# HasnainRaz/Fast-SRGAN

Hardware: AMD Instinct MI355X
Metric: SR train-step images/sec (96->384 4x, full GAN step: G+D+VGG perceptual loss) (higher is better)
Workload: dtype x3v; 1 GPU; BASELINE configs[2]: full GAN training step, 8 residual blocks / 64 filters, 96x96->384x384; per_gpu_batch=32, global_batch=32, parallelism=dp1, collectives=none, rccl_world_size=1, launch=hipGraph replay

## Files before the change

fast-srgan_amd/_lib.py:

```python
import ctypes
import os

_HERE = os.path.dirname(os.path.abspath(__file__))
LIB_PATH = os.environ.get("FSR_HIP_LIB") or os.path.join(_HERE, "libfsr_hip.so")

FSR_F32, FSR_BF16, FSR_F16, FSR_X3 = 0, 1, 2, 3
ACT_NONE, ACT_RELU, ACT_LEAKY, ACT_PRELU, ACT_TANH = 0, 1, 2, 3, 4
CONV_FWD, CONV_DGRAD = 0, 1
PACK_FWD, PACK_FWD_PS, PACK_DGRAD, PACK_DGRAD_PS = 0, 1, 2, 3
OUT_DTYPE, OUT_F32, OUT_U8, OUT_I420, OUT_NV12 = 0, 1, 2, 3, 4
YUV_BT601, YUV_BT709 = 0, 1
SITING_JPEG, SITING_MPEG2 = 0, 1
CHROMA_420, CHROMA_422, CHROMA_444 = 0, 1, 2
LAYOUT_PLANAR, LAYOUT_NV12 = 0, 1
BLUR_MAX_RADIUS, BLUR_TAPS = 9, 19
QUALITY_Y, QUALITY_RGB = 0, 1
OPT_BIAS, OPT_PRELU, OPT_OSCALE, OPT_MASK, OPT_PREACT, OPT_STATS = 1, 2, 4, 8, 16, 32
ABI_VERSION = 16

c_int, c_float, c_void_p, c_size_t, c_ll = ctypes.c_int, ctypes.c_float, ctypes.c_void_p, ctypes.c_size_t, ctypes.c_longlong


class ConvDesc(ctypes.Structure):
    _fields_ = [
# ... 44 lines not shown
    "fsr_i420_to_image_deep": (c_int, [P, P, c_int, c_int, c_int, c_int, c_int, c_int, c_int, P]),
    "fsr_image_to_i420": (c_int, [P, c_int, c_int, c_int, c_int, c_int, c_int, P, P]),
    "fsr_resample_image_i420_deep": (c_int, [P, c_int, c_int, c_int, c_int, c_int, P, P, P, c_int, P, P, P, c_int, c_int, c_int, c_int, P, P]),
    "fsr_yuv_to_image": (c_int, [P, P, c_int, c_int, c_int, c_int, c_int, c_int, c_int, c_int, P]),
    "fsr_image_to_yuv": (c_int, [P, c_int, c_int, c_int, c_int, c_int, c_int, c_int, P, P]),
    "fsr_resample_image_yuv": (c_int, [P, c_int, c_int, c_int, c_int, c_int, P, P, P, c_int, P, P, P, c_int, c_int, c_int, c_int, c_int, P, P]),
    "fsr_yuv_to_image_ex": (c_int, [P, P, c_int, c_int, c_int, c_int, c_int, c_int, c_int, c_int, c_int, P]),
    "fsr_image_to_yuv_ex": (c_int, [P, c_int, c_int, c_int, c_int, c_int, c_int, c_int, c_int, P, P]),
    "fsr_resample_image_yuv_ex": (c_int, [P, c_int, c_int, c_int, c_int, c_int, P, P, P, c_int, P, P, P, c_int, c_int, c_int, c_int, c_int, c_int,
                                          P, P]),
    "fsr_resample_image": (c_int, [P, c_int, c_int, c_int, c_int, c_int, P, P, P, c_int, P, P, P, c_int, c_int, c_int, c_int, P, P]),
    "fsr_pack_conv3x3_c3": (c_int, [c_int, P, c_int, P, c_int, P]),
    "fsr_tanh_bwd_image": (c_int, [P, c_ll, c_ll, c_ll, c_ll, P, c_int, c_int, c_int, P, P, P, P]),
    "fsr_conv3x3_c3_fwd": (c_int, [c_int, P, c_ll, c_ll, c_ll, c_ll, c_int, c_int, c_int, c_float, c_float, c_float, c_float,
                                   c_float, c_float, P, P, c_int, c_float, P, c_int, P, P, P, P]),
    "fsr_conv3x3_c3_wgrad_workspace": (ctypes.c_size_t, [c_int, c_int, c_int, c_int]),
    "fsr_conv3x3_c3_wgrad": (c_int, [c_int, P, c_ll, c_ll, c_ll, c_ll, c_int, c_int, c_int, c_float, c_float, c_float,
                                     c_float, c_float, c_float, P, c_int, P, P, P, c_int, P]),
    "fsr_tanh_bwd_scratch": (c_size_t, []),
    "fsr_tanh_bwd_to_nhwc": (c_int, [c_int, P, c_ll, c_ll, c_ll, c_ll, P, c_int, c_int, c_int, P, c_int, P, P, P]),
    "fsr_maxpool2_fwd": (c_int, [c_int, P, P, P, c_int, c_int, c_int, c_int, P]),
    "fsr_png_to_npy": (c_int, [P, P, c_int, c_int, P]),
    "fsr_png_decode_chw": (c_int, [ctypes.c_char_p, P, c_size_t, P, P]),
    "fsr_maxpool2_bwd_argmax": (c_int, [c_int, P, P, P, c_int, c_int, c_int, c_int, c_int, P]),
    "fsr_maxpool2_bwd": (c_int, [c_int, P, P, P, P, c_int, c_int, c_int, c_int, c_int, P]),
    "fsr_conv1x1_c1_fwd": (c_int, [c_int, P, P, P, P, c_int, c_int, P]),
    "fsr_conv1x1_c1_bwd_scratch": (c_size_t, [c_int]),
    "fsr_conv1x1_c1_bwd": (c_int, [c_int, P, P, P, P, P, P, P, c_int, c_int, P]),
    "fsr_loss_scratch": (c_size_t, []),
    "fsr_bce_logits_fwd": (c_int, [P, P, P, P, c_ll, P]),
# ... 66 lines not shown
```

fast-srgan_amd/csrc/conv_c3.hip:

```cpp
#include "fsr_common.h"
#include "fsr_host.h"

namespace {

struct C3Args {
  const float* img;
  long long sn, sc, sh, sw;
  int N, H, W;
  float scale[3], shift[3];
  const void* wpk;
  const float* bias;
  const float* prelu;
  int act;
  float slope;
  int cout;
  void* out;
  void* preact;
  unsigned char* signs;
  const void* dz;
  float* ws;
  int tiles_x, tiles_y, tiles_per_slab, ntiles;
};

constexpr int PW = 18;

__device__ __forceinline__ int patch_off(int k) {
  const int tap = k / 3, ci = k - tap * 3;
  return ((tap / 3) * PW + (tap % 3)) * 3 + ci;
}

template <typename T> __device__ __forceinline__ float round_T(float v);
template <> __device__ __forceinline__ float round_T<float>(float v) { return v; }
template <> __device__ __forceinline__ float round_T<bf16_t>(float v) { return bf2f(f2bf(v)); }
template <> __device__ __forceinline__ float round_T<f16_t>(float v) { return (float)(f16_t)v; }

#ifndef FSR_ABLC3
#define FSR_ABLC3 0
#endif
constexpr int C3_ABL = FSR_ABLC3;
#if FSR_ABLC3
#define C3_KEEP(v) asm volatile("" ::"v"(v))
#else
#define C3_KEEP(v) ((void)0)
#endif

template <int TH> struct PatchRegs {
  static constexpr int PN = (TH + 2) * PW * 3;
  static constexpr int PPT = (PN + 255) / 256;
  float v[PPT];
  unsigned okmask;
};
template <int TH>
__device__ __forceinline__ void patch_load(const C3Args& a, PatchRegs<TH>& r, int n, int y0, int x0, int tid) {
  const float* src = a.img + n * a.sn;
// ... 47 lines not shown
    const bool ok = i < PN && y >= 0 && y < a.H && x >= 0 && x < a.W;
    okmask |= (ok ? 1u : 0u) << j;
    if constexpr ((C3_ABL & 8) != 0) v[j] = (float)(i & 15);
    else v[j] = src[ok ? ci * a.sc + y * a.sh + x * a.sw : 0];
  }
#pragma unroll
  for (int j = 0; j < PPT; ++j) {
    const int i = tid + j * 256;
    const int ci = i % 3;
    const float sc = ci == 0 ? a.scale[0] : (ci == 1 ? a.scale[1] : a.scale[2]);
    const float sh = ci == 0 ? a.shift[0] : (ci == 1 ? a.shift[1] : a.shift[2]);
    if (i < PN) patch[i] = ((okmask >> j) & 1u) ? round_T<T>(v[j] * sc + sh) : 0.f;
  }
}

template <typename T, typename ST = T, int ROWS = 16>
__global__ __launch_bounds__(256) void conv_c3_fwd_kernel(const C3Args a) {
  constexpr int TH = ROWS, RPW = ROWS / 4;
  constexpr int PN = (TH + 2) * PW * 3, PPT = (PN + 255) / 256;
  constexpr bool STRIP = ROWS > 16;
  static_assert(ROWS == 16 || ROWS == 32 || ROWS == 64, "strip height");
  __shared__ float patch[PN];
  const int tid = threadIdx.x, lane = tid & 63, wave = __builtin_amdgcn_readfirstlane(tid >> 6);
  const int l15 = lane & 15, lg = lane >> 4;
  int bid = blockIdx.x;
  const int tx = bid % a.tiles_x;
  bid /= a.tiles_x;
  const int ty = bid % a.tiles_y;
  const int n = bid / a.tiles_y;
  const int nb = blockIdx.y;
  const int ntile = (a.cout - nb * 64 >= 64) ? 4 : (a.cout - nb * 64) / 16;
// ... 15 lines not shown
      if constexpr ((C3_ABL & 8) != 0) pv[j] = (float)(i & 15);
      else pv[j] = src[ok ? (unsigned)ci * usc + (unsigned)y * ush + (unsigned)x * usw : 0u];
    }
  }

  const T* wpk = (const T*)a.wpk;
  int koff[8];
  if constexpr (sizeof(T) == 2) {
#pragma unroll
    for (int e = 0; e < 8; ++e) koff[e] = (8 * lg + e < 27) ? patch_off(8 * lg + e) : -1;
  } else {
#pragma unroll
    for (int j = 0; j < 8; ++j) koff[j] = (lg + 4 * j < 27) ? patch_off(lg + 4 * j) : -1;
  }
  constexpr bool X3 = std::is_same<ST, x3_t>::value;
  const bool wide = (sizeof(T) == 2 || X3) && ntile == 4;
  s16x8 wf16[4];
  float wf32[4][8];
#pragma unroll
  for (int t = 0; t < 4; ++t) {
    if (t < ntile) {
      const int ch = wide ? (t >> 1) * 32 + (l15 >> 2) * 8 + (t & 1) * 4 + (l15 & 3) : t * 16 + l15;
      const T* row = wpk + (size_t)(nb * 64 + ch) * 32;
      if constexpr ((C3_ABL & 16) != 0) {
        if constexpr (sizeof(T) == 2) {
          wf16[t] = (s16x8){(short)lane, (short)t, 1, 2, 3, 4, 5, 6};
        } else {
#pragma unroll
          for (int j = 0; j < 8; ++j) wf32[t][j] = (float)(lane + j);
        }
      } else if constexpr (sizeof(T) == 2) {
        wf16[t] = *(const s16x8*)(row + 8 * lg);
      } else {
#pragma unroll
        for (int j = 0; j < 8; ++j) wf32[t][j] = row[lg + 4 * j];
      }
    }
  }
  float slope = (a.act == FSR_ACT_PRELU) ? a.prelu[0] : a.slope;
  if (a.act == FSR_ACT_NONE) slope = 1.f;
  if (a.act == FSR_ACT_RELU) slope = 0.f;
  f32x4 bv[4];
#pragma unroll
  for (int i = 0; i < 4; ++i) bv[i] = (f32x4){0.f, 0.f, 0.f, 0.f};
  auto load_bias = [&]() {
    if (a.bias) {
      if (wide) {
#pragma unroll
        for (int p = 0; p < 2; ++p) {
          bv[2 * p] = *(const f32x4*)(a.bias + nb * 64 + p * 32 + lg * 8);
          bv[2 * p + 1] = *(const f32x4*)(a.bias + nb * 64 + p * 32 + lg * 8 + 4);
        }
      } else {
#pragma unroll
        for (int t = 0; t < 4; ++t)
          if (t < ntile) bv[t] = *(const f32x4*)(a.bias + nb * 64 + t * 16 + lg * 4);
// ... 19 lines not shown
  if constexpr (!STRIP) load_bias();
#pragma unroll 1
  for (int m0 = 0; m0 < RPW; m0 += 4) {
    int mo = m0;
    if constexpr (STRIP) {
      FSR_TOUCH(mo);
      mo = __builtin_amdgcn_readfirstlane(mo);
    }
#pragma unroll
  for (int m = 0; m < 4; ++m) {
    const int r = wave * RPW + mo + m;
    const int gy = ty * TH + r;
    if constexpr (STRIP) {
      if (gy >= a.H) break;
    }
    const float* base = patch + (r * PW + l15) * 3;
    float xv[8];
#pragma unroll
    for (int e = 0; e < 8; ++e) xv[e] = koff[e] >= 0 ? base[koff[e]] : 0.f;
    s16x8 xf16;
    if constexpr (sizeof(T) == 2) {
      const unsigned p0 = pack2<T>(xv[0], xv[1]), p1 = pack2<T>(xv[2], xv[3]);
      const unsigned p2 = pack2<T>(xv[4], xv[5]), p3 = pack2<T>(xv[6], xv[7]);
      xf16 = __builtin_bit_cast(s16x8, (u32x4){p0, p1, p2, p3});
    }
    if constexpr (sizeof(T) == 2) {
      if (wide) {
        f32x4 acc[4];
#pragma unroll
        for (int t = 0; t < 4; ++t) {
// ... 3 lines not shown
        if (gx < a.W && gy < a.H) {
          const size_t off = (((size_t)n * a.H + gy) * a.W + gx) * a.cout + nb * 64 + lg * 8;
#pragma unroll
          for (int p = 0; p < 2; ++p) {
            f32x4 lo = acc[2 * p], hi = acc[2 * p + 1];
            lo += bv[2 * p];
            hi += bv[2 * p + 1];
            if (prep)
              fsr_st<4>((u32x4*)((T*)prep + off + p * 32), (u32x4)((u32x4){pack2<T>(lo[0], lo[1]), pack2<T>(lo[2], lo[3]),
                                                       pack2<T>(hi[0], hi[1]), pack2<T>(hi[2], hi[3])}));
#pragma unroll
            for (int q = 0; q < 4; ++q) {
              lo[q] = fmaxf(lo[q], 0.f) + slope * fminf(lo[q], 0.f);
              hi[q] = fmaxf(hi[q], 0.f) + slope * fminf(hi[q], 0.f);
            }
            const u32x4 pk = (u32x4){pack2<T>(lo[0], lo[1]), pack2<T>(lo[2], lo[3]), pack2<T>(hi[0], hi[1]), pack2<T>(hi[2], hi[3])};
            if constexpr ((C3_ABL & 1) != 0) C3_KEEP(pk);
            else fsr_st<4>((u32x4*)((T*)outp + off + p * 32), pk);
            if (a.signs) {
              unsigned b = 0u;
#pragma unroll
              for (int q = 0; q < 4; ++q) b |= ((int)(pk[q] << 16) > 0 ? 1u << (2 * q) : 0u) | ((int)(pk[q] & 0xffff0000u) > 0 ? 2u << (2 * q) : 0u);
              a.signs[(((size_t)n * a.H + gy) * a.W + gx) * (a.cout >> 3) + nb * 8 + p * 4 + lg] = (unsigned char)b;
            }
          }
        }
        continue;
      }
    }
    if constexpr (X3) {
      if (wide) {
// ... 4 lines not shown
#pragma unroll
          for (int j = 0; j < 8; ++j) {
            if constexpr ((C3_ABL & 2) != 0) acc[t][j & 3] += wf32[t][j] + xv[j];
            else acc[t] = mfma_f32_16x16x4(wf32[t][j], xv[j], acc[t]);
          }
        }
        if (gx < a.W && gy < a.H) {
          const size_t off = (((size_t)n * a.H + gy) * a.W + gx) * a.cout + nb * 64 + lg * 8;
#pragma unroll
          for (int p = 0; p < 2; ++p) {
            const f32x4 lo = acc[2 * p] + bv[2 * p], hi = acc[2 * p + 1] + bv[2 * p + 1];
            float v8[8] = {lo[0], lo[1], lo[2], lo[3], hi[0], hi[1], hi[2], hi[3]};
            if (prep) V16<x3_t, 4>::st((x3_t*)prep + off + p * 32, v8);
#pragma unroll
            for (int q = 0; q < 8; ++q) v8[q] = fmaxf(v8[q], 0.f) + slope * fminf(v8[q], 0.f);
            if constexpr ((C3_ABL & 1) != 0) {
#pragma unroll
              for (int q = 0; q < 8; ++q) C3_KEEP(v8[q]);
            } else {
              V16<x3_t, 4>::st((x3_t*)outp + off + p * 32, v8);
            }
            if (a.signs) {
              unsigned b = 0u;
#pragma unroll
              for (int q = 0; q < 4; ++q) {
                const unsigned hh = pack_bf16x2(v8[2 * q], v8[2 * q + 1]);
                b |= ((int)(hh << 16) > 0 ? 1u << (2 * q) : 0u) | ((int)(hh & 0xffff0000u) > 0 ? 2u << (2 * q) : 0u);
              }
              a.signs[(((size_t)n * a.H + gy) * a.W + gx) * (a.cout >> 3) + nb * 8 + p * 4 + lg] = (unsigned char)b;
            }
// ... 33 lines not shown
          if constexpr (sizeof(T) == 2) {
            u32x2 pk;
            pk.x = pack2<T>(acc[0], acc[1]);
            pk.y = pack2<T>(acc[2], acc[3]);
            fsr_st<4>((u32x2*)((T*)outp + off), (u32x2)(pk));
          } else if constexpr (std::is_same<ST, x3_t>::value) {
            x3_st4(outp + off, acc);
          } else {
            *(f32x4*)(outp + off) = acc;
          }
        }
      }
    });
  }
  }
}

template <typename T, typename ST = T>
__global__ __launch_bounds__(256) void conv_c3_wgrad_kernel(const C3Args a) {
  constexpr int TH = 8;
  constexpr bool F32 = sizeof(T) == 4;
  constexpr int PA = F32 ? 64 : 64 + 16;
  constexpr int PN = (TH + 2) * PW * 3;
  __shared__ float patch[PN];
  __shared__ __attribute__((aligned(16))) T dzt[TH * 16 * PA];
  const int tid = threadIdx.x, lane = tid & 63, wave = __builtin_amdgcn_readfirstlane(tid >> 6);
  const int l15 = lane & 15, lg = lane >> 4;
  const int slab = blockIdx.x, nb = blockIdx.y;
  const int cvalid = a.cout - nb * 64;
  const bool active = wave * 16 < cvalid;
  const ST* dzg = (const ST*)a.dz;
// ... 194 lines not shown
  }
  if (dtype != FSR_X3 || preact) return 16;
  const long long tiles_x = (w + 15) / 16;
  for (int rows = 64; rows > 16; rows >>= 1) {
    const long long strips = (h + rows - 1) / rows;
    if (tiles_x * strips * n >= C3_FWD_MIN_ROUNDS * C3_FWD_SLOTS && (strips * rows - h) * C3_FWD_MAX_PAD <= h) return rows;
  }
  return 16;
}

template <typename T, typename ST>
void c3_fwd_launch(int rows, dim3 grid, hipStream_t stream, const C3Args& a) {
  if (rows == 64) hipLaunchKernelGGL((conv_c3_fwd_kernel<T, ST, 64>), grid, dim3(256), 0, stream, a);
  else if (rows == 32) hipLaunchKernelGGL((conv_c3_fwd_kernel<T, ST, 32>), grid, dim3(256), 0, stream, a);
  else hipLaunchKernelGGL((conv_c3_fwd_kernel<T, ST, 16>), grid, dim3(256), 0, stream, a);
}

}

extern "C" int fsr_pack_conv3x3_c3(int dtype, const float* w_oihw, int cout, void* packed, int transposed, fsr_stream_t stream_) {
  if (!w_oihw || !packed || cout <= 0) return fsr_fail(-1, "fsr_pack_conv3x3_c3: bad argument");
  const int rows_pad = (cout + 15) / 16 * 16;
  const int blocks = (rows_pad * 32 + 255) / 256;
  if (dtype == FSR_BF16)
    hipLaunchKernelGGL(pack_c3_kernel<bf16_t>, dim3(blocks), dim3(256), 0, (hipStream_t)stream_, w_oihw, (bf16_t*)packed, cout, rows_pad, transposed);
  else if (dtype == FSR_F16)
    hipLaunchKernelGGL(pack_c3_kernel<f16_t>, dim3(blocks), dim3(256), 0, (hipStream_t)stream_, w_oihw, (f16_t*)packed, cout, rows_pad, transposed);
  else if (dtype == FSR_F32 || dtype == FSR_X3)
    hipLaunchKernelGGL(pack_c3_kernel<float>, dim3(blocks), dim3(256), 0, (hipStream_t)stream_, w_oihw, (float*)packed, cout, rows_pad, transposed);
  else
// ... 23 lines not shown
  a.signs = (unsigned char*)signs;
  const int rows = c3_fwd_rows(dtype, preact != nullptr, n, h, w, sc, sh, sw);
  a.tiles_x = (w + 15) / 16;
  a.tiles_y = (h + rows - 1) / rows;
  const long long nwg = (long long)a.tiles_x * a.tiles_y * n;
  if (nwg > 0x7fffffffLL) return fsr_fail(-2, "fsr_conv3x3_c3_fwd: bad grid");
  const dim3 grid((unsigned)nwg, (unsigned)((cout + 63) / 64));
  const hipStream_t stream = (hipStream_t)stream_;
  if (dtype == FSR_BF16) c3_fwd_launch<bf16_t, bf16_t>(rows, grid, stream, a);
  else if (dtype == FSR_F16) c3_fwd_launch<f16_t, f16_t>(rows, grid, stream, a);
  else if (dtype == FSR_X3) c3_fwd_launch<float, x3_t>(rows, grid, stream, a);
  else c3_fwd_launch<float, float>(rows, grid, stream, a);
  return fsr_check_launch("conv_c3_fwd_kernel");
}

static int c3_wgrad_slabs(int n, int h, int w, int* tiles_x, int* tiles_y, int* per) {
  *tiles_x = (w + 15) / 16;
  *tiles_y = (h + 7) / 8;
  const long long ntiles = (long long)*tiles_x * *tiles_y * n;
  long long want = 1024;
  if (want > ntiles) want = ntiles;
  *per = (int)((ntiles + want - 1) / want);
  return (int)((ntiles + *per - 1) / *per);
}

extern "C" size_t fsr_conv3x3_c3_wgrad_workspace(int n, int h, int w, int cout) {
  int tx, ty, per;
  if (n <= 0 || h <= 0 || w <= 0 || cout <= 0) return 0;
  return (size_t)c3_wgrad_slabs(n, h, w, &tx, &ty, &per) * cout * 32 * sizeof(float);
}
// ... 25 lines not shown
```

fast-srgan_amd/model.py:

```python
import os
import warnings

import torch

from . import _lib as L
from . import ops

_DEFAULT_DTYPE = os.environ.get("FSR_COMPUTE_DTYPE", "f16")


def split_compute_dtype(name):
    if name == "x3v":
        return "x3", "f16"
    return name, name


class UpSamplingBlock(torch.nn.Module):

    def __init__(self, config):
        super().__init__()
        self.conv = torch.nn.Conv2d(config.n_filters, config.n_filters * 4, kernel_size=3, padding=1)
        self.phase_shift = torch.nn.PixelShuffle(upscale_factor=2)
        self.relu = torch.nn.PReLU()

# ... 17 lines not shown
        self.compute = ops.Compute(split_compute_dtype(compute_dtype or _DEFAULT_DTYPE)[0])
        if nf % self.compute.cpad:
            raise ValueError("n_filters=%d must be a multiple of %d in %s mode" % (nf, self.compute.cpad, self.compute.name))
        self.neck = torch.nn.Sequential(torch.nn.Conv2d(3, nf, kernel_size=3, padding=1), torch.nn.PReLU())
        self.stem = torch.nn.Sequential(*[ResidualBlock(nf, nf) for _ in range(config.n_layers)])
        self.bottleneck = torch.nn.Sequential(
            torch.nn.Conv2d(nf, nf, kernel_size=3, padding=1, bias=False), torch.nn.InstanceNorm2d(nf))
        self.upsampling = torch.nn.Sequential(*[UpSamplingBlock(config) for _ in range(getattr(config, "n_upsample", 2))])
        self.head = torch.nn.Sequential(torch.nn.Conv2d(nf, 3, kernel_size=3, padding=1), torch.nn.Tanh())
        cd = self.compute
        self._cfg_neck = ops.ConvCfg(cd, act=L.ACT_PRELU, image_in=True)
        self._cfg_in = ops.ConvCfg(cd, stats=True)
        self._cfg_in_skip = ops.ConvCfg(cd, stats=True, n_alias=1)
        self._cfg_in_skip2 = ops.ConvCfg(cd, stats=True, n_alias=2)
        self._cfg_up = ops.ConvCfg(cd, act=L.ACT_PRELU, pixel_shuffle=True)
        self._cfg_head = ops.ConvCfg(cd, tanh_head=True)
        self._cfg_head_u8 = ops.ConvCfg(cd, tanh_head=True, u8_head=True)
        self._cfg_head_i420 = {}

    def _native_size(self, h, w, out_size):
        if out_size is None:
            return True
        s = 2 ** len(self.upsampling)
        oh, ow = out_size
        if int(oh) != oh or int(ow) != ow or oh <= 0 or ow <= 0:
            raise ValueError("out_size must be (out_h, out_w) of positive integers, got %r" % (out_size,))
        return (int(oh), int(ow)) == (s * h, s * w)

    def forward_u8(self, frames, out_size=None, bands=None, ensemble=False):
        with torch.no_grad():
# ... 69 lines not shown
            x = ops.dihedral_members(frames, g0, g0 + 3)
            for k0 in range(g0, g0 + 4, per):
                k1 = min(k0 + per, g0 + 4) - 1
                y = self._forward(x[(k0 - g0) * n:(k1 - g0 + 1) * n], self._cfg_head, bands)
                out = ops.dihedral_accumulate(y.permute(0, 2, 3, 1), k0, k1, acc, kind)
        return out

    def _forward(self, x, cfg_head, bands=None):
        m = self._body(x)
        if bands is None or not len(self.upsampling):
            return self._tail(m, cfg_head)
        return self._tail_banded(m, cfg_head, bands)

    def _tail(self, m, cfg_head):
        for up in list(self.upsampling)[-1:]:
            m, _ = ops.conv3x3(m, up.conv.weight, up.conv.bias, up.relu.weight, self._cfg_up)
        out, _ = ops.conv3x3(m, self.head[0].weight, self.head[0].bias, None, cfg_head)
        return out

    def _tail_banded(self, m, cfg_head, bands):
        R = int(bands)
        if isinstance(bands, bool) or R != bands or R < 1:
            raise ValueError("bands must be None or the number of core rows per band (an integer >= 1), got %r" % (bands,))
        if torch.is_grad_enabled():
            raise L.FsrError("bands: the banded tail is inference-only (it has no gradient); call it under torch.no_grad()")
        n, H2, W2, c = m.shape
        wins = ops.tail_windows(H2, R)
        if len(wins) == 1:
            return self._tail(m, cfg_head)
        Hw, total = R + 2 * ops.TAIL_HALO, n * len(wins)
        cup = self.upsampling[-1].conv.out_channels
# ... 196 lines not shown
```

fast-srgan_amd/ops.py:

```python
import ctypes
import math
import os
import weakref

import numpy as np
import torch

from . import _lib as L

_DT = {"f32": (L.FSR_F32, torch.float32, 16), "bf16": (L.FSR_BF16, torch.bfloat16, 32), "f16": (L.FSR_F16, torch.float16, 32),
       "x3": (L.FSR_X3, torch.float32, 32)}


class Compute:

    def __init__(self, name="f16"):
        if name not in _DT:
            raise ValueError("compute dtype must be 'bf16', 'f16', 'x3' or 'f32', got %r" % (name,))
        self.name = name
        self.code, self.torch_dtype, self.cpad = _DT[name]
        self.x3 = name == "x3"
        self.pack_dtype = torch.bfloat16 if self.x3 else self.torch_dtype
        self.pack_kmul = 2 if self.x3 else 1
        self.is16 = name in ("bf16", "f16")
# ... 217 lines not shown

def _const_vec(values, device):
    key = (tuple(values), str(device))
    t = _const.get(key)
    if t is None:
        t = torch.tensor(values, dtype=torch.float32, device=device)
        _const[key] = t
    return t

USE_LIN_PACK = os.environ.get("FSR_PACK_LIN", "1") != "0"
USE_SIGN_BITS = os.environ.get("FSR_SIGN_BITS", "1") != "0" and os.environ.get("FSR_S2D3", "1") != "0"
_pack_block_memo = {}
_DISPATCH_ENV = ("FSR_PERSIST_CUS", "FSR_T3_ROWS", "FSR_S2D3", "FSR_T3N_G3", "FSR_CONV_STAGE", "FSR_CONV64_S2FWD",
                 "FSR_PACK_LIN")
USE_POOL_ARGMAX = os.environ.get("FSR_POOL_ARGMAX", "1") != "0"
USE_C3_KERNELS = True

PROFILE_CONV = None


def _last_kernel():
    name = L.lib().fsr_last_kernel()
    return name.decode() if name else "?"


_ws_retired = []
_capture_seen = {}


def _workspace(nbytes, device):
# ... 201 lines not shown
        img = img.float()
    n, c, h, w = img.shape
    if c != 3:
        raise ValueError("expected a 3-channel image batch, got %s" % (tuple(img.shape),))
    out = _empty((n, h, w, cd.cpad), cd.torch_dtype, img.device)
    sn, sc, sh, sw = img.stride()
    L.check(L.lib().fsr_image_to_nhwc(cd.code, _p(img), sn, sc, sh, sw, n, h, w, scale[0], scale[1], scale[2], shift[0],
                                      shift[1], shift[2], _p(out), cd.cpad, _stream()), "fsr_image_to_nhwc")
    return out


class ConvCfg:

    def __init__(self, cd, *, stride=1, act=L.ACT_NONE, slope=0.0, pixel_shuffle=False, stats=False, image_in=False,
                 in_scale=(1.0, 1.0, 1.0), in_shift=(0.0, 0.0, 0.0), tanh_head=False, input_act_bwd=None,
                 act_bwd_by_consumer=False, u8_head=False, pool_after=False, n_alias=0, emit_signs=False, i420_head=None):
        self.input_act_bwd, self.act_bwd_by_consumer = input_act_bwd, act_bwd_by_consumer
        self.cd, self.stride, self.act, self.slope = cd, stride, act, slope
        self.pixel_shuffle, self.stats, self.image_in = pixel_shuffle, stats, image_in
        self.in_scale, self.in_shift, self.tanh_head = in_scale, in_shift, tanh_head
        self.u8_head = u8_head and tanh_head
        self.i420_head = i420_head if tanh_head else None
        self.pool_after = pool_after
        self.n_alias = n_alias
        self.emit_signs = emit_signs


class Conv3x3Fn(torch.autograd.Function):

    @staticmethod
    def forward(ctx, x, weight, bias, prelu, cfg, grad_on=True):
        ctx.grad_on = grad_on
        cd = cfg.cd
        cout, cin = weight.shape[0], weight.shape[1]
        if (cfg.image_in and cfg.stride == 1 and cout % 16 == 0 and not (cfg.pixel_shuffle or cfg.stats or cfg.tanh_head)
                and USE_C3_KERNELS):
            return Conv3x3Fn._forward_c3(ctx, x, weight, bias, prelu, cfg)
        ctx.c3 = False
        ctx.in_signs = getattr(x, "_fsr_signs", None) if (cfg.input_act_bwd is not None and cfg.stride == 2 and (cd.is16 or cd.x3)) else None
        if cfg.image_in:
            xin = image_to_nhwc(cd, x, cfg.in_scale, cfg.in_shift)
        else:
            xin = x if x.is_contiguous() else x.contiguous()
            if xin.dtype != cd.torch_dtype:
                raise L.FsrError("activation dtype %s does not match the module's compute dtype %s" % (xin.dtype, cd.name))
        cin_pad = xin.shape[3]
        wpk = FilterSpec(weight, L.PACK_FWD_PS if cfg.pixel_shuffle else L.PACK_FWD, cin_pad)
        training = ctx.grad_on and any(ctx.needs_input_grad)
        if (cfg.u8_head or cfg.i420_head or cfg.pool_after) and training:
            raise L.FsrError("the uint8 / I420 head and fused max-pool epilogues are inference-only: they have no gradient")
        act = L.ACT_TANH if cfg.tanh_head else cfg.act
        want_pre = training and act == L.ACT_PRELU
        b32 = bias if bias is None or bias.dtype == torch.float32 else bias.float()
        out, pre, stats = conv3x3_raw(cd, xin, wpk, cout, stride=cfg.stride, bias=b32, act=act, slope=cfg.slope,
                                      prelu=prelu, pixel_shuffle=cfg.pixel_shuffle, out_f32=cfg.tanh_head,
                                      want_stats=cfg.stats, want_preact=want_pre, alg_k=cin, out_u8=cfg.u8_head,
                                      pool2=cfg.pool_after, out_i420=cfg.i420_head)
        ctx.cfg = cfg
        ctx.dims = (cout, cin, tuple(xin.shape))
        ctx.has_bias = bias is not None
        ctx.x_is_image = cfg.image_in
        saved_act = pre if want_pre else (out if act in (L.ACT_RELU, L.ACT_LEAKY, L.ACT_TANH) else None)
        ctx.save_for_backward(xin, weight, prelu, saved_act)
        if stats is None:
            stats = torch.empty(0, device=out.device)
        ctx.mark_non_differentiable(stats)
        ctx.set_materialize_grads(False)
        if cfg.u8_head or cfg.i420_head:
            return out, stats
        if cfg.tanh_head:
            return out.permute(0, 3, 1, 2), stats
        if cfg.n_alias:
            if cfg.image_in or cfg.input_act_bwd is not None or cfg.pixel_shuffle or cfg.stride != 1:
                raise L.FsrError("skip aliases are for plain stride-1 convolutions on NHWC activations")
            return (out, stats) + tuple(xin.view_as(xin) for _ in range(cfg.n_alias))
        return out, stats

    @staticmethod
# ... 62 lines not shown
        if cfg.tanh_head:
            if g.dtype != torch.float32:
                g = g.float()
            _, _, h, w = g.shape
            dz = _empty((n, h, w, cd.cpad), cd.torch_dtype, xin.device)
            sn, sc, sh, sw = g.stride()
            L.check(lib.fsr_tanh_bwd_to_nhwc(cd.code, _p(g), sn, sc, sh, sw, _p(saved), n, h, w, _p(dz), cd.cpad, _p(dbias),
                                             _p(_workspace(lib.fsr_tanh_bwd_scratch(), xin.device)), st), "fsr_tanh_bwd_to_nhwc")
        else:
            g = g if g.is_contiguous() else g.contiguous()
            if cd.x3:
                g, saved = _aligned(g), _aligned(saved)
            bias_arena = getattr(getattr(ctx, "bias_param", None), "_fsr_grad", None) if ctx.c3 else None
            fused_dbias = (bias_arena is not None and cfg.act_bwd_by_consumer and ctx.needs_input_grad[1] and ctx.needs_input_grad[2]
                           and getattr(weight, "_fsr_grad", None) is not None)
            if cfg.act_bwd_by_consumer:
                dz = g
                if ctx.has_bias and ctx.needs_input_grad[2] and not fused_dbias:
                    _, h, w, c = g.shape
                    scr = _workspace(lib.fsr_act_bwd_scratch(n, h, w, c, int(cfg.pixel_shuffle)), xin.device)
                    L.check(lib.fsr_act_bwd(cd.code, _p(g), None, L.ACT_NONE, 0.0, None, None, _p(dbias), None, _p(scr), n, h, w,
                                            c, int(cfg.pixel_shuffle), st), "fsr_act_bwd")
            elif act != L.ACT_NONE or ctx.has_bias:
                if act == L.ACT_PRELU:
                    dprelu = _zeros((1,), xin.device)
                dz = _empty_like(g)
                _, h, w, c = g.shape
                scr = _workspace(lib.fsr_act_bwd_scratch(n, h, w, c, int(cfg.pixel_shuffle)), xin.device)
                L.check(lib.fsr_act_bwd(cd.code, _p(g), _p(saved), act, float(cfg.slope), _p(prelu), _p(dz), _p(dbias),
                                        _p(dprelu), _p(scr), n, h, w, c, int(cfg.pixel_shuffle), st), "fsr_act_bwd")
            else:
# ... 62 lines not shown
    if g.dtype != torch.float32:
        g = g.float()
    if cd.x3:
        xin = _aligned(xin)
    dbias = _zeros((cout,), xin.device) if (ctx.has_bias and ctx.needs_input_grad[2]) else None
    dz_img = torch.empty((n, ih, iw, 3), dtype=torch.float32, device=xin.device)
    sn, sc, sh, sw = g.stride()
    L.check(lib.fsr_tanh_bwd_image(_p(g), sn, sc, sh, sw, _p(saved), n, ih, iw, _p(dz_img), _p(dbias),
                                   _p(_workspace(lib.fsr_tanh_bwd_scratch(), xin.device)), st), "fsr_tanh_bwd_image")
    img_strides = (ih * iw * 3, 1, iw * 3, 3)
    one, zero = (1.0, 1.0, 1.0), (0.0, 0.0, 0.0)
    dx = None
    if ctx.needs_input_grad[0]:
        wpk = packed_filter(cd, weight, PACK_C3T, 32)
        dx = _empty((n, ih, iw, cin_pad), cd.torch_dtype, xin.device)
        prof = PROFILE_CONV
        if prof is not None:
            ev0, ev1 = torch.cuda.Event(enable_timing=True), torch.cuda.Event(enable_timing=True)
            ev0.record()
        L.check(lib.fsr_conv3x3_c3_fwd(cd.code, _p(dz_img), *img_strides, n, ih, iw, *one, *zero, _p(wpk), None, L.ACT_NONE, 0.0, None,
                                       cin_pad, _p(dx), None, None, st), "fsr_conv3x3_c3_fwd")
        if prof is not None:
            ev1.record()
            prof.append((ev0, ev1, 2.0 * n * ih * iw * cin * 27, dz_img.numel() * 4 + dx.numel() * dx.element_size(), "conv_c3_fwd_kernel", "dgrad"))
    dw = None
    if ctx.needs_input_grad[1]:
        arena = getattr(weight, "_fsr_grad", None)

        def launch():
            out = arena if arena is not None else torch.zeros((cout, cin, 3, 3), dtype=torch.float32, device=xin.device)
            need = lib.fsr_conv3x3_c3_wgrad_workspace(n, ih, iw, cin_pad)
            L.check(lib.fsr_conv3x3_c3_wgrad(cd.code, _p(dz_img), *img_strides, n, ih, iw, *one, *zero, _p(xin), cin_pad, _p(out), None,
                                             _p(_workspace(need, xin.device)), 1, _stream()), "fsr_conv3x3_c3_wgrad")
            return out

        if arena is not None:
            with _on_wgrad_stream(xin, dz_img):
                launch()
        else:
# ... 646 lines not shown
```

include/fsr_hip.h:

```cpp
#ifndef FSR_HIP_H
#define FSR_HIP_H

#include <stddef.h>
#include <stdint.h>

#ifdef __cplusplus
extern "C" {
#endif

#define FSR_ABI_VERSION 16

enum { FSR_F32 = 0, FSR_BF16 = 1, FSR_F16 = 2, FSR_X3 = 3 };
enum { FSR_ACT_NONE = 0, FSR_ACT_RELU = 1, FSR_ACT_LEAKY = 2, FSR_ACT_PRELU = 3, FSR_ACT_TANH = 4 };
enum { FSR_CONV_FWD = 0, FSR_CONV_DGRAD = 1 };
enum { FSR_PACK_FWD = 0, FSR_PACK_FWD_PS = 1, FSR_PACK_DGRAD = 2, FSR_PACK_DGRAD_PS = 3 };
enum { FSR_OUT_DTYPE = 0, FSR_OUT_F32 = 1, FSR_OUT_U8 = 2, FSR_OUT_I420 = 3, FSR_OUT_NV12 = 4 };
enum { FSR_YUV_BT601 = 0, FSR_YUV_BT709 = 1 };
enum { FSR_SITING_JPEG = 0, FSR_SITING_MPEG2 = 1 };
enum { FSR_CHROMA_420 = 0, FSR_CHROMA_422 = 1, FSR_CHROMA_444 = 2 };
enum { FSR_LAYOUT_PLANAR = 0, FSR_LAYOUT_NV12 = 1 };

typedef void* fsr_stream_t;

int fsr_version(void);
// ... 98 lines not shown
int fsr_resample_image_i420_deep(const float* t, int n, int h, int w, int oh, int ow, const float* wy, const int* ymin, const int* ysize,
                                 int ky, const float* wx, const int* xmin, const int* xsize, int kx, int yuv_matrix, int yuv_full_range,
                                 int depth, void* out, fsr_stream_t stream);
int fsr_resample_image_yuv(const float* t, int n, int h, int w, int oh, int ow, const float* wy, const int* ymin, const int* ysize, int ky,
                           const float* wx, const int* xmin, const int* xsize, int kx, int chroma, int yuv_matrix, int yuv_full_range,
                           int depth, void* out, fsr_stream_t stream);
int fsr_resample_image_yuv_ex(const float* t, int n, int h, int w, int oh, int ow, const float* wy, const int* ymin, const int* ysize, int ky,
                              const float* wx, const int* xmin, const int* xsize, int kx, int chroma, int layout, int yuv_matrix,
                              int yuv_full_range, int depth, void* out, fsr_stream_t stream);

int fsr_pack_conv3x3_c3(int dtype, const float* w_oihw, int cout, void* packed, int transposed, fsr_stream_t stream);
int fsr_conv3x3_c3_fwd(int dtype, const float* img, long long sn, long long sc, long long sh, long long sw, int n, int h,
                       int w, float scale0, float scale1, float scale2, float shift0, float shift1, float shift2,
                       const void* packed_w, const float* bias, int act, float slope, const float* prelu_weight, int cout,
                       void* out, void* preact, void* signs, fsr_stream_t stream);
size_t fsr_conv3x3_c3_wgrad_workspace(int n, int h, int w, int cout);
int fsr_conv3x3_c3_wgrad(int dtype, const float* img, long long sn, long long sc, long long sh, long long sw, int n, int h,
                         int w, float scale0, float scale1, float scale2, float shift0, float shift1, float shift2,
                         const void* dz, int cout, float* dw_oihw, float* dbias, void* workspace, int transposed,
                         fsr_stream_t stream);

int fsr_maxpool2_fwd(int dtype, const void* x, void* y, void* argmax, int n, int h, int w, int c, fsr_stream_t stream);
int fsr_maxpool2_bwd_argmax(int dtype, const void* g, const void* argmax, void* dx, int n, int h, int w, int c, int relu_mask,
                            fsr_stream_t stream);
int fsr_maxpool2_bwd(int dtype, const void* g, const void* x, const void* y, void* dx, int n, int h, int w, int c,
                     int relu_mask, fsr_stream_t stream);

int fsr_conv1x1_c1_fwd(int dtype, const void* x, const float* w, const float* b, float* logits, int npix, int c,
                       fsr_stream_t stream);
size_t fsr_conv1x1_c1_bwd_scratch(int c);
// ... 77 lines not shown
```

Before: 609.6 images/s.

## Fuse PReLU backward into tanh-head dgrad conv for last upsampling layer

```diff
diff --git a/fast-srgan_amd/_lib.py b/fast-srgan_amd/_lib.py
--- a/fast-srgan_amd/_lib.py
+++ b/fast-srgan_amd/_lib.py
@@ -82,6 +82,8 @@
     "fsr_tanh_bwd_image": (c_int, [P, c_ll, c_ll, c_ll, c_ll, P, c_int, c_int, c_int, P, P, P, P]),
     "fsr_conv3x3_c3_fwd": (c_int, [c_int, P, c_ll, c_ll, c_ll, c_ll, c_int, c_int, c_int, c_float, c_float, c_float, c_float,
                                    c_float, c_float, P, P, c_int, c_float, P, c_int, P, P, P, P]),
+    "fsr_conv3x3_c3_dgrad_act_scratch": (c_size_t, [c_int, c_int, c_int, c_int]),
+    "fsr_conv3x3_c3_dgrad_act": (c_int, [c_int, P, c_ll, c_ll, c_ll, c_ll, c_int, c_int, c_int, P, c_int, P, P, P, P, c_int, P, P]),
     "fsr_conv3x3_c3_wgrad_workspace": (ctypes.c_size_t, [c_int, c_int, c_int, c_int]),
     "fsr_conv3x3_c3_wgrad": (c_int, [c_int, P, c_ll, c_ll, c_ll, c_ll, c_int, c_int, c_int, c_float, c_float, c_float,
                                      c_float, c_float, c_float, P, c_int, P, P, P, c_int, P]),
diff --git a/fast-srgan_amd/csrc/conv_c3.hip b/fast-srgan_amd/csrc/conv_c3.hip
--- a/fast-srgan_amd/csrc/conv_c3.hip
+++ b/fast-srgan_amd/csrc/conv_c3.hip
@@ -20,6 +20,9 @@
   const void* dz;
   float* ws;
   int tiles_x, tiles_y, tiles_per_slab, ntiles;
+  const void* dact_pre;
+  const float* dact_slope;
+  double* dact_part;
 };
 
 constexpr int PW = 18;
@@ -38,6 +41,10 @@
 #define FSR_ABLC3 0
 #endif
 constexpr int C3_ABL = FSR_ABLC3;
+#ifndef FSR_C3_DACT_AHEAD
+#define FSR_C3_DACT_AHEAD 1
+#endif
+constexpr bool C3_DACT_AHEAD = FSR_C3_DACT_AHEAD != 0;
 #if FSR_ABLC3
 #define C3_KEEP(v) asm volatile("" ::"v"(v))
 #else
@@ -115,7 +122,13 @@
   }
 }
 
-template <typename T, typename ST = T, int ROWS = 16>
+__device__ __forceinline__ double shfl_xor_f64(double v, int m) {
+  const u32x2 w = __builtin_bit_cast(u32x2, v);
+  const u32x2 r = {(unsigned)__shfl_xor((int)w.x, m, 64), (unsigned)__shfl_xor((int)w.y, m, 64)};
+  return __builtin_bit_cast(double, r);
+}
+
+template <typename T, typename ST = T, int ROWS = 16, bool DACT = false>
 __global__ __launch_bounds__(256) void conv_c3_fwd_kernel(const C3Args a) {
   constexpr int TH = ROWS, RPW = ROWS / 4;
   constexpr int PN = (TH + 2) * PW * 3, PPT = (PN + 255) / 256;
@@ -161,7 +174,8 @@
     for (int j = 0; j < 8; ++j) koff[j] = (lg + 4 * j < 27) ? patch_off(lg + 4 * j) : -1;
   }
   constexpr bool X3 = std::is_same<ST, x3_t>::value;
-  const bool wide = (sizeof(T) == 2 || X3) && ntile == 4;
+  static_assert(!DACT || sizeof(T) == 2 || X3, "the fused activation backward has 16-bit and x3 forms");
+  const bool wide = DACT || ((sizeof(T) == 2 || X3) && ntile == 4);
   s16x8 wf16[4];
   float wf32[4][8];
 #pragma unroll
@@ -187,6 +201,28 @@
   float slope = (a.act == FSR_ACT_PRELU) ? a.prelu[0] : a.slope;
   if (a.act == FSR_ACT_NONE) slope = 1.f;
   if (a.act == FSR_ACT_RELU) slope = 0.f;
+  float dslope = 1.f;
+  double dp = 0.0;
+  u32x4 nh[2], nl[X3 ? 2 : 1];
+  auto pre_issue = [&](int r) {
+    const int gy = ty * TH + r, px = tx * 16 + l15;
+    const bool ok = r < (wave + 1) * RPW && gy < a.H && px < a.W;
+    const size_t off = ok ? (((size_t)n * a.H + gy) * a.W + px) * a.cout + nb * 64 + lg * 8 : 0;
+#pragma unroll
+    for (int p = 0; p < 2; ++p) {
+      if constexpr (X3) {
+        const char* hp = (const char*)x3_hi_ptr((const x3_t*)a.dact_pre + off + p * 32);
+        nh[p] = *FSR_GLOBAL_PTR(const u32x4, hp);
+        nl[p] = *FSR_GLOBAL_PTR(const u32x4, hp + 64);
+      } else {
+        nh[p] = *FSR_GLOBAL_PTR(const u32x4, (const T*)a.dact_pre + off + p * 32);
+      }
+    }
+  };
+  if constexpr (DACT) {
+    dslope = a.dact_slope[0];
+    if constexpr (C3_DACT_AHEAD) pre_issue(wave * RPW);
+  }
   f32x4 bv[4];
 #pragma unroll
   for (int i = 0; i < 4; ++i) bv[i] = (f32x4){0.f, 0.f, 0.f, 0.f};
@@ -236,6 +272,16 @@
     if constexpr (STRIP) {
       if (gy >= a.H) break;
     }
+    u32x4 ch[2], cl[X3 ? 2 : 1];
+    if constexpr (DACT) {
+      if constexpr (!C3_DACT_AHEAD) pre_issue(r);
+#pragma unroll
+      for (int p = 0; p < 2; ++p) {
+        ch[p] = nh[p];
+        if constexpr (X3) cl[p] = nl[p];
+      }
+      if constexpr (C3_DACT_AHEAD) pre_issue(r + 1);
+    }
     const float* base = patch + (r * PW + l15) * 3;
     float xv[8];
 #pragma unroll
@@ -269,7 +315,20 @@
               lo[q] = fmaxf(lo[q], 0.f) + slope * fminf(lo[q], 0.f);
               hi[q] = fmaxf(hi[q], 0.f) + slope * fminf(hi[q], 0.f);
             }
-            const u32x4 pk = (u32x4){pack2<T>(lo[0], lo[1]), pack2<T>(lo[2], lo[3]), pack2<T>(hi[0], hi[1]), pack2<T>(hi[2], hi[3])};
+            u32x4 pk = (u32x4){pack2<T>(lo[0], lo[1]), pack2<T>(lo[2], lo[3]), pack2<T>(hi[0], hi[1]), pack2<T>(hi[2], hi[3])};
+            if constexpr (DACT) {
+#pragma unroll
+              for (int q = 0; q < 4; ++q) {
+                const float g0 = cvt_lo<T>(pk[q]), g1 = cvt_hi<T>(pk[q]);
+                const float z0 = cvt_lo<T>(ch[p][q]), z1 = cvt_hi<T>(ch[p][q]);
+                dp += (double)g0 * (double)fminf(z0, 0.f);
+                dp += (double)g1 * (double)fminf(z1, 0.f);
+                float d0 = g0 * (z0 > 0.f ? 1.f : dslope), d1 = g1 * (z1 > 0.f ? 1.f : dslope);
+                FSR_TOUCH(d0);
+                FSR_TOUCH(d1);
+                pk[q] = pack2<T>(d0, d1);
+              }
+            }
             if constexpr ((C3_ABL & 1) != 0) C3_KEEP(pk);
             else fsr_st<4>((u32x4*)((T*)outp + off + p * 32), pk);
             if (a.signs) {
@@ -304,6 +363,21 @@
             if (prep) V16<x3_t, 4>::st((x3_t*)prep + off + p * 32, v8);
 #pragma unroll
             for (int q = 0; q < 8; ++q) v8[q] = fmaxf(v8[q], 0.f) + slope * fminf(v8[q], 0.f);
+            if constexpr (DACT) {
+#pragma unroll
+              for (int i = 0; i < 4; ++i) {
+                unsigned hh, ll;
+                x3_split2(v8[2 * i], v8[2 * i + 1], hh, ll);
+                const float g0 = x3_join_lo(hh, ll), g1 = x3_join_hi(hh, ll);
+                const float z0 = x3_join_lo(ch[p][i], cl[p][i]), z1 = x3_join_hi(ch[p][i], cl[p][i]);
+                dp += (double)g0 * (double)fminf(z0, 0.f);
+                dp += (double)g1 * (double)fminf(z1, 0.f);
+                v8[2 * i] = g0 * (z0 > 0.f ? 1.f : dslope);
+                v8[2 * i + 1] = g1 * (z1 > 0.f ? 1.f : dslope);
+                FSR_TOUCH(v8[2 * i]);
+                FSR_TOUCH(v8[2 * i + 1]);
+              }
+            }
             if constexpr ((C3_ABL & 1) != 0) {
 #pragma unroll
               for (int q = 0; q < 8; ++q) C3_KEEP(v8[q]);
@@ -367,7 +441,30 @@
     });
   }
   }
-}
+  if constexpr (DACT) {
+    __shared__ double red_p[4];
+#pragma unroll
+    for (int o = 32; o >= 1; o >>= 1) dp += shfl_xor_f64(dp, o);
+    if (lane == 0) red_p[wave] = dp;
+    __syncthreads();
+    if (tid == 0) a.dact_part[blockIdx.y * gridDim.x + blockIdx.x] = ((red_p[0] + red_p[1]) + red_p[2]) + red_p[3];
+  }
+}
+
+__global__ __launch_bounds__(256) void conv_c3_dact_reduce_kernel(const double* __restrict__ part, int nwg, float* __restrict__ dprelu, int accumulate) {
+  __shared__ double red[256];
+  const int tid = threadIdx.x;
+  double s = 0.0;
+  for (int i = tid; i < nwg; i += 256) s += part[i];
+  red[tid] = s;
+  __syncthreads();
+  for (int o = 128; o >= 1; o >>= 1) {
+    if (tid < o) red[tid] += red[tid + o];
+    __syncthreads();
+  }
+  if (tid == 0) dprelu[0] = accumulate ? dprelu[0] + (float)red[0] : (float)red[0];
+}
+
 
 template <typename T, typename ST = T>
 __global__ __launch_bounds__(256) void conv_c3_wgrad_kernel(const C3Args a) {
@@ -592,6 +689,27 @@
   if (rows == 64) hipLaunchKernelGGL((conv_c3_fwd_kernel<T, ST, 64>), grid, dim3(256), 0, stream, a);
   else if (rows == 32) hipLaunchKernelGGL((conv_c3_fwd_kernel<T, ST, 32>), grid, dim3(256), 0, stream, a);
   else hipLaunchKernelGGL((conv_c3_fwd_kernel<T, ST, 16>), grid, dim3(256), 0, stream, a);
+}
+
+int c3_dgrad_act_rows(int dtype, int n, int h, int w, long long sc, long long sh, long long sw) {
+  const int rows = c3_fwd_rows(dtype, false, n, h, w, sc, sh, sw);
+  if (sc < 0 || sh < 0 || sw < 0 || 2 * sc + (long long)(h - 1) * sh + (long long)(w - 1) * sw >= (1LL << 31)) return rows;
+  if (const char* e = getenv("FSR_C3_DGRAD_ROWS")) {
+    const int f = atoi(e);
+    if (f == 16 || f == 32 || f == 64) return f;
+  }
+  return rows;
+}
+
+template <typename T, typename ST>
+void c3_dgrad_act_launch(int rows, dim3 grid, hipStream_t stream, const C3Args& a) {
+  if (rows == 64) hipLaunchKernelGGL((conv_c3_fwd_kernel<T, ST, 64, true>), grid, dim3(256), 0, stream, a);
+  else if (rows == 32) hipLaunchKernelGGL((conv_c3_fwd_kernel<T, ST, 32, true>), grid, dim3(256), 0, stream, a);
+  else hipLaunchKernelGGL((conv_c3_fwd_kernel<T, ST, 16, true>), grid, dim3(256), 0, stream, a);
+}
+
+long long c3_dgrad_act_slots(int n, int h, int w, int cout) {
+  return (long long)((w + 15) / 16) * ((h + 15) / 16) * n * (cout / 64);
 }
 
 }
@@ -645,6 +763,43 @@
   return fsr_check_launch("conv_c3_fwd_kernel");
 }
 
+extern "C" size_t fsr_conv3x3_c3_dgrad_act_scratch(int n, int h, int w, int cout) {
+  if (n <= 0 || h <= 0 || w <= 0 || cout <= 0 || cout % 64) return 0;
+  return (size_t)c3_dgrad_act_slots(n, h, w, cout) * sizeof(double);
+}
+
+extern "C" int fsr_conv3x3_c3_dgrad_act(int dtype, const float* img, long long sn, long long sc, long long sh, long long sw, int n,
+                                        int h, int w, const void* packed_w, int cout, const void* preact, const float* prelu_weight,
+                                        void* dz, float* dprelu, int accumulate, void* scratch, fsr_stream_t stream_) {
+  C3Args a = {};
+  const float one3[3] = {1.f, 1.f, 1.f}, zero3[3] = {0.f, 0.f, 0.f};
+  if (int rc = fill_args(a, "fsr_conv3x3_c3_dgrad_act", dtype, img, sn, sc, sh, sw, n, h, w, one3, zero3, cout)) return rc;
+  if (!packed_w || !preact || !prelu_weight || !dz || !dprelu || !scratch) return fsr_fail(-1, "fsr_conv3x3_c3_dgrad_act: null argument");
+  if (dtype == FSR_F32) return fsr_fail(-2, "fsr_conv3x3_c3_dgrad_act: 16-bit dtypes and FSR_X3 only");
+  if (cout % 64) return fsr_fail(-2, "fsr_conv3x3_c3_dgrad_act: cout=%d is not a multiple of 64", cout);
+  if (dtype == FSR_X3 && ((((size_t)dz | (size_t)preact) & 127) != 0)) return fsr_fail(-2, "fsr_conv3x3_c3_dgrad_act: x3 tensors must be 128-byte aligned");
+  a.wpk = packed_w;
+  a.act = FSR_ACT_NONE;
+  a.out = dz;
+  a.dact_pre = preact;
+  a.dact_slope = prelu_weight;
+  if ((size_t)scratch & 7) return fsr_fail(-2, "fsr_conv3x3_c3_dgrad_act: scratch must be 8-byte aligned");
+  a.dact_part = (double*)scratch;
+  const int rows = c3_dgrad_act_rows(dtype, n, h, w, sc, sh, sw);
+  a.tiles_x = (w + 15) / 16;
+  a.tiles_y = (h + rows - 1) / rows;
+  const long long nwg = (long long)a.tiles_x * a.tiles_y * n * (cout / 64);
+  if (nwg > c3_dgrad_act_slots(n, h, w, cout) || nwg > 0x7fffffffLL) return fsr_fail(-2, "fsr_conv3x3_c3_dgrad_act: bad grid");
+  const dim3 grid((unsigned)(nwg / (cout / 64)), (unsigned)(cout / 64));
+  const hipStream_t stream = (hipStream_t)stream_;
+  if (dtype == FSR_BF16) c3_dgrad_act_launch<bf16_t, bf16_t>(rows, grid, stream, a);
+  else if (dtype == FSR_F16) c3_dgrad_act_launch<f16_t, f16_t>(rows, grid, stream, a);
+  else c3_dgrad_act_launch<float, x3_t>(rows, grid, stream, a);
+  if (int rc = fsr_check_launch("conv_c3_fwd_kernel<dact>")) return rc;
+  hipLaunchKernelGGL(conv_c3_dact_reduce_kernel, dim3(1), dim3(256), 0, stream, (const double*)a.dact_part, (int)nwg, dprelu, accumulate ? 1 : 0);
+  return fsr_check_launch("conv_c3_dact_reduce_kernel");
+}
+
 static int c3_wgrad_slabs(int n, int h, int w, int* tiles_x, int* tiles_y, int* per) {
   *tiles_x = (w + 15) / 16;
   *tiles_y = (h + 7) / 8;
diff --git a/fast-srgan_amd/model.py b/fast-srgan_amd/model.py
--- a/fast-srgan_amd/model.py
+++ b/fast-srgan_amd/model.py
@@ -55,6 +55,7 @@
         self._cfg_in_skip = ops.ConvCfg(cd, stats=True, n_alias=1)
         self._cfg_in_skip2 = ops.ConvCfg(cd, stats=True, n_alias=2)
         self._cfg_up = ops.ConvCfg(cd, act=L.ACT_PRELU, pixel_shuffle=True)
+        self._cfg_up_last = ops.ConvCfg(cd, act=L.ACT_PRELU, pixel_shuffle=True, offer_act_bwd=True)
         self._cfg_head = ops.ConvCfg(cd, tanh_head=True)
         self._cfg_head_u8 = ops.ConvCfg(cd, tanh_head=True, u8_head=True)
         self._cfg_head_i420 = {}
@@ -154,7 +155,7 @@
 
     def _tail(self, m, cfg_head):
         for up in list(self.upsampling)[-1:]:
-            m, _ = ops.conv3x3(m, up.conv.weight, up.conv.bias, up.relu.weight, self._cfg_up)
+            m, _ = ops.conv3x3(m, up.conv.weight, up.conv.bias, up.relu.weight, self._cfg_up_last)
         out, _ = ops.conv3x3(m, self.head[0].weight, self.head[0].bias, None, cfg_head)
         return out
 
diff --git a/fast-srgan_amd/ops.py b/fast-srgan_amd/ops.py
--- a/fast-srgan_amd/ops.py
+++ b/fast-srgan_amd/ops.py
@@ -255,6 +255,7 @@
 _DISPATCH_ENV = ("FSR_PERSIST_CUS", "FSR_T3_ROWS", "FSR_S2D3", "FSR_T3N_G3", "FSR_CONV_STAGE", "FSR_CONV64_S2FWD",
                  "FSR_PACK_LIN")
 USE_POOL_ARGMAX = os.environ.get("FSR_POOL_ARGMAX", "1") != "0"
+USE_C3_DGRAD_ACT = os.environ.get("FSR_C3_DGRAD_ACT", "1") != "0"
 USE_C3_KERNELS = True
 
 PROFILE_CONV = None
@@ -486,7 +487,8 @@
 
     def __init__(self, cd, *, stride=1, act=L.ACT_NONE, slope=0.0, pixel_shuffle=False, stats=False, image_in=False,
                  in_scale=(1.0, 1.0, 1.0), in_shift=(0.0, 0.0, 0.0), tanh_head=False, input_act_bwd=None,
-                 act_bwd_by_consumer=False, u8_head=False, pool_after=False, n_alias=0, emit_signs=False, i420_head=None):
+                 act_bwd_by_consumer=False, u8_head=False, pool_after=False, n_alias=0, emit_signs=False, i420_head=None,
+                 offer_act_bwd=False):
         self.input_act_bwd, self.act_bwd_by_consumer = input_act_bwd, act_bwd_by_consumer
         self.cd, self.stride, self.act, self.slope = cd, stride, act, slope
         self.pixel_shuffle, self.stats, self.image_in = pixel_shuffle, stats, image_in
@@ -496,6 +498,13 @@
         self.pool_after = pool_after
         self.n_alias = n_alias
         self.emit_signs = emit_signs
+        self.offer_act_bwd = offer_act_bwd
+
+
+class _ActTicket:
+
+    def __init__(self, pre, prelu):
+        self.pre, self.prelu, self.taken, self.dprelu = pre, prelu, False, None
 
 
 class Conv3x3Fn(torch.autograd.Function):
@@ -510,6 +519,7 @@
             return Conv3x3Fn._forward_c3(ctx, x, weight, bias, prelu, cfg)
         ctx.c3 = False
         ctx.in_signs = getattr(x, "_fsr_signs", None) if (cfg.input_act_bwd is not None and cfg.stride == 2 and (cd.is16 or cd.x3)) else None
+        ctx.in_ticket = getattr(x, "_fsr_act_bwd", None) if (cfg.tanh_head and USE_C3_DGRAD_ACT) else None
         if cfg.image_in:
             xin = image_to_nhwc(cd, x, cfg.in_scale, cfg.in_shift)
         else:
@@ -534,6 +544,9 @@
         ctx.x_is_image = cfg.image_in
         saved_act = pre if want_pre else (out if act in (L.ACT_RELU, L.ACT_LEAKY, L.ACT_TANH) else None)
         ctx.save_for_backward(xin, weight, prelu, saved_act)
+        ctx.act_ticket = None
+        if cfg.offer_act_bwd and want_pre and USE_C3_DGRAD_ACT and (cd.is16 or cd.x3) and not cfg.n_alias:
+            ctx.act_ticket = out._fsr_act_bwd = _ActTicket(pre, prelu)
         if stats is None:
             stats = torch.empty(0, device=out.device)
         ctx.mark_non_differentiable(stats)
@@ -626,7 +639,10 @@
             bias_arena = getattr(getattr(ctx, "bias_param", None), "_fsr_grad", None) if ctx.c3 else None
             fused_dbias = (bias_arena is not None and cfg.act_bwd_by_consumer and ctx.needs_input_grad[1] and ctx.needs_input_grad[2]
                            and getattr(weight, "_fsr_grad", None) is not None)
-            if cfg.act_bwd_by_consumer:
+            ticket = getattr(ctx, "act_ticket", None)
+            if ticket is not None and ticket.taken and ticket.dprelu is not None:
+                dprelu = ticket.dprelu
+            if cfg.act_bwd_by_consumer or (ticket is not None and ticket.taken):
                 dz = g
                 if ctx.has_bias and ctx.needs_input_grad[2] and not fused_dbias:
                     _, h, w, c = g.shape
@@ -719,15 +735,29 @@
     if ctx.needs_input_grad[0]:
         wpk = packed_filter(cd, weight, PACK_C3T, 32)
         dx = _empty((n, ih, iw, cin_pad), cd.torch_dtype, xin.device)
+        ticket = getattr(ctx, "in_ticket", None)
+        if ticket is not None and not ((cd.is16 or cd.x3) and cin_pad % 64 == 0 and tuple(ticket.pre.shape) == (n, ih, iw, cin_pad)):
+            ticket = None
         prof = PROFILE_CONV
         if prof is not None:
             ev0, ev1 = torch.cuda.Event(enable_timing=True), torch.cuda.Event(enable_timing=True)
             ev0.record()
-        L.check(lib.fsr_conv3x3_c3_fwd(cd.code, _p(dz_img), *img_strides, n, ih, iw, *one, *zero, _p(wpk), None, L.ACT_NONE, 0.0, None,
-                                       cin_pad, _p(dx), None, None, st), "fsr_conv3x3_c3_fwd")
+        if ticket is not None:
+            pre = _aligned(ticket.pre) if cd.x3 else ticket.pre
+            arena = getattr(ticket.prelu, "_fsr_grad", None)
+            ticket.dprelu = None if arena is not None else _assigned((1,), xin.device)
+            scr = _workspace(lib.fsr_conv3x3_c3_dgrad_act_scratch(n, ih, iw, cin_pad), xin.device)
+            L.check(lib.fsr_conv3x3_c3_dgrad_act(cd.code, _p(dz_img), *img_strides, n, ih, iw, _p(wpk), cin_pad, _p(pre), _p(ticket.prelu), _p(dx),
+                                                 _p(arena if arena is not None else ticket.dprelu), int(arena is not None), _p(scr), st),
+                    "fsr_conv3x3_c3_dgrad_act")
+            ticket.taken = True
+        else:
+            L.check(lib.fsr_conv3x3_c3_fwd(cd.code, _p(dz_img), *img_strides, n, ih, iw, *one, *zero, _p(wpk), None, L.ACT_NONE, 0.0, None,
+                                           cin_pad, _p(dx), None, None, st), "fsr_conv3x3_c3_fwd")
         if prof is not None:
             ev1.record()
-            prof.append((ev0, ev1, 2.0 * n * ih * iw * cin * 27, dz_img.numel() * 4 + dx.numel() * dx.element_size(), "conv_c3_fwd_kernel", "dgrad"))
+            prof.append((ev0, ev1, 2.0 * n * ih * iw * cin * 27, dz_img.numel() * 4 + dx.numel() * dx.element_size() * (2 if ticket is not None else 1),
+                         "conv_c3_fwd_kernel", "dgrad"))
     dw = None
     if ctx.needs_input_grad[1]:
         arena = getattr(weight, "_fsr_grad", None)
diff --git a/include/fsr_hip.h b/include/fsr_hip.h
--- a/include/fsr_hip.h
+++ b/include/fsr_hip.h
@@ -136,6 +136,10 @@
                        int w, float scale0, float scale1, float scale2, float shift0, float shift1, float shift2,
                        const void* packed_w, const float* bias, int act, float slope, const float* prelu_weight, int cout,
                        void* out, void* preact, void* signs, fsr_stream_t stream);
+size_t fsr_conv3x3_c3_dgrad_act_scratch(int n, int h, int w, int cout);
+int fsr_conv3x3_c3_dgrad_act(int dtype, const float* img, long long sn, long long sc, long long sh, long long sw, int n, int h,
+                             int w, const void* packed_w, int cout, const void* preact, const float* prelu_weight, void* dz,
+                             float* dprelu, int accumulate, void* scratch, fsr_stream_t stream);
 size_t fsr_conv3x3_c3_wgrad_workspace(int n, int h, int w, int cout);
 int fsr_conv3x3_c3_wgrad(int dtype, const float* img, long long sn, long long sc, long long sh, long long sw, int n, int h,
                          int w, float scale0, float scale1, float scale2, float shift0, float shift1, float shift2,
```

Measured after the change: 612.5 images/s, median of 6. No clear change (+0.5%).
